# MingXiangL/SPE

Hardware: AMD Instinct MI355X
Metric: images/sec (whole node) at 3x800x1333 bs=2/GPU (higher is better)
Workload: dtype bf16/fp16 operands, fp32 accumulate; 1 GPU; TSCAM_cait_S24 (C=384, depth 24, 8 heads) + 0-layer encoder + 6-layer conditional-DETR decoder x2 stages, 100 queries, COCO heads (91), 2x3x800x1333 per GPU (N=4150 tokens), fwd + SetCriterion + SetCriterionRefine + bwd + grad all-reduce + clip + AdamW; global_batch=2, parallelism=dp1

## Files before the change

include/spe_hip.h:

```cpp
#ifndef SPE_HIP_H
#define SPE_HIP_H
#include <stddef.h>
#include <stdint.h>

#ifdef __cplusplus
extern "C" {
#endif

typedef struct ihipStream_t* spe_stream_t;

int spe_abi_version(void);

int spe_set_reduce_workspace(void* ws, size_t bytes, spe_stream_t stream);
int spe_reduce_defer_ranges(const void* const* ptrs, const size_t* bytes, int n);
int spe_reduce_defer_arena(void* arena, size_t bytes);
int spe_reduce_flush(spe_stream_t stream);
int spe_reduce_pending(void);

int spe_gemm_f32(const float* A, const float* B, float* C, const float* bias, float* C2,
                 int M, int N, int K, long lda, long ldb, long ldc, int transA, int transB,
                 int batch0, int batch1, long sA0, long sA1, long sB0, long sB1, long sC0, long sC1,
                 float alpha, int act, int splitk, int precision, spe_stream_t stream);

int spe_gemm_ex(const void* A, int a_bf16, const float* B, float* C, const float* bias, float* C2,
// ... 28 lines not shown
                               float* const* db, int R, int nblk, int N, int K, spe_stream_t stream);
int spe_gemm_bf16tn(const void* A16, const void* B16, float* C, int M, int N, int R, long lda, long ldb, long ldc,
                    float alpha, int splitk, spe_stream_t stream);
int spe_gemm_bf16tn_plan(int M, int N, int R, long lda, long ldb, int splitk, int* v);
int spe_gemm_bf16nt_ex(const void* A16, const void* B16, const void* A16lo, const void* B16lo, float* C, const float* bias,
                       float* C2, void* out16, void* out16lo, long ld16, void* out16T, long ld16t, float* colsum, const float* aux,
                       const float* res, const float* rgamma, int M, int N, int K, long lda, long ldb, long ldc, float alpha, int act,
                       int half_flags, spe_stream_t stream);
int spe_gemm_bf16nt_exd(const void* A16, const void* B16, const void* A16lo, const void* B16lo, float* C, const float* bias,
                        float* C2, void* out16, void* out16lo, long ld16, void* out16T, long ld16t, float* colsum, const float* aux,
                        const float* res, const float* rgamma, int M, int N, int K, long lda, long ldb, long ldc, float alpha, int act,
                        int half_flags, float p_drop, uint64_t seed, uint64_t offset, const float* sample_scale, long rows_per_sample,
                        spe_stream_t stream);
int spe_gemm_bf16nt_plan(int M, int N, int K, int split, int ex, int f16_operands, int f16_second, int splitk, int has_out16t,
                         long ld16t, int* plan);
int spe_cvt_bf16(const float* x, long ldx, int R, int C, void* out, void* out_lo, long ldo, void* outT, long ldt, float* colsum,
                 const float* aux, int act, spe_stream_t stream);
int spe_cvt_bf16_h(const float* x, long ldx, int R, int C, void* out, void* out_h, long ldo, void* outT, long ldt, spe_stream_t stream);
int spe_cvt_bf16_multi(const void* jobs_dev, int njobs, int total_tiles, spe_stream_t stream);

int spe_softmax_fwd(const float* S, const unsigned char* mask, float* P, float* Pd, int B, int H, int Nq,
                    int Nk, long ld, float p_drop, uint64_t seed, uint64_t offset, spe_stream_t stream);
int spe_softmax_bwd(const float* dPd, const float* P, float* dS, int B, int H, int Nq, int Nk, long ld,
                    float p_drop, uint64_t seed, uint64_t offset, spe_stream_t stream);

int spe_talking_softmax_fwd(const float* S, const float* Wl, const float* bl, const float* Ww, const float* bw,
                            float* P, float* Pd, int B, int H, int Nq, int Nk, long ld, float p_drop,
                            uint64_t seed, uint64_t offset, spe_stream_t stream);
int spe_talking_softmax_bwd(const float* dPd, const float* P, const float* S, const float* Wl, const float* Ww,
                            float* dS, float* ws, int nblocks, int B, int H, int Nq, int Nk, long ld,
// ... 158 lines not shown
```

spe_amd/csrc/gemm_bf16.hip:

```cpp
#include <cstdlib>
#include "common.h"
#include "gemm16_epilogue.h"
#include "det_reduce.h"
#include "gemm_nt_select.h"
#include "gemm_tiles.h"

template <int R>
__device__ __forceinline__ void g16_load(const unsigned short* __restrict__ base, long ld, int row0, int nrows, int k0, int K,
                                         u32x4g_t (&v)[R / 32]) {
    const int t = threadIdx.x;
    const int k = k0 + (t & 7) * 8;
    const bool kv = k < K;
    const int kc = kv ? k : 0;
#pragma unroll
    for (int i = 0; i < R / 32; ++i) {
        const int r = min(row0 + (t >> 3) + 32 * i, nrows - 1);
        const u32x4g_t q = *reinterpret_cast<const u32x4g_t*>(base + (long)r * ld + kc);
        v[i] = kv ? q : (u32x4g_t){0u, 0u, 0u, 0u};
    }
}
template <int R>
__device__ __forceinline__ void g16_stage(unsigned short* lds, const u32x4g_t (&v)[R / 32]) {
    const int t = threadIdx.x;
#pragma unroll
// ... 233 lines not shown
    p.out16 = nullptr; p.out16T = nullptr; p.colsum = nullptr; p.aux = nullptr; p.ld16 = 0; p.ld16t = 0; p.res = nullptr; p.rgamma = nullptr;
    p.drop_p = 0.f; p.drop_seed = p.drop_off = 0; p.sscale = nullptr; p.rps = 1;
    const int ktiles = (K + GB_BK - 1) / GB_BK;
    if (p.h16 && (splitk != 1 || C2 || (ldc & 3))) return -2;
    if ((p.h16 & 1) && A16lo) return -2;
    if (splitk < 0) {
        splitk = -splitk; p.slab = (long)M * ldc;
        if (splitk > ktiles) return -5;
    } else if (splitk > 1) return -2;
    if (splitk < 1) splitk = 1;
    p.kt_per_split = (ktiles + splitk - 1) / splitk;
    p.splitk = splitk;
    if (splitk > 1 && (act != 0 || C2 != nullptr || bias != nullptr)) return -3;
    if (p.Alo && splitk != 1) return -3;
    return nt_gemm_launch(p, false, stream);
}

static int gemm_bf16nt_ex_impl(const void* A16, const void* B16, const void* A16lo, const void* B16lo, float* C, const float* bias,
                               float* C2, void* out16, void* out16lo, long ld16, void* out16T, long ld16t, float* colsum,
                               const float* aux, const float* res, const float* rgamma,
                               int M, int N, int K, long lda, long ldb, long ldc, float alpha, int act, int half_flags,
                               float p_drop, uint64_t seed, uint64_t offset, const float* sample_scale, long rows_per_sample, hipStream_t stream);
extern "C" int spe_gemm_bf16nt_ex(const void* A16, const void* B16, const void* A16lo, const void* B16lo, float* C, const float* bias,
                                  float* C2, void* out16, void* out16lo, long ld16, void* out16T, long ld16t, float* colsum,
                                  const float* aux, const float* res, const float* rgamma,
                                  int M, int N, int K, long lda, long ldb, long ldc, float alpha, int act, int half_flags, hipStream_t stream) {
    return gemm_bf16nt_ex_impl(A16, B16, A16lo, B16lo, C, bias, C2, out16, out16lo, ld16, out16T, ld16t, colsum, aux, res, rgamma, M, N, K, lda, ldb,
                               ldc, alpha, act, half_flags, 0.f, 0, 0, nullptr, 1, stream);
}
extern "C" int spe_gemm_bf16nt_exd(const void* A16, const void* B16, const void* A16lo, const void* B16lo, float* C, const float* bias,
// ... 194 lines not shown
```

spe_amd/csrc/gemm_nt2.hip:

```cpp
#include <cstdlib>
#include "common.h"
#include "gemm16_epilogue.h"
#include "gemm_nt_select.h"
#include "gemm_tiles.h"

template <int CPR>
__device__ __forceinline__ int nt2_swz(int r) {
    if constexpr (CPR == 8) return r & 7;
    else return (0x78 >> (2 * ((r >> 2) & 3))) & 3;
}

template <int BM, int BN, int BK, int NST, bool SPLIT, bool EX, bool F16>
__global__ __launch_bounds__(256, 2) void gemm_nt2_kernel(Gemm16Args p) {
    extern __shared__ __attribute__((aligned(16))) unsigned short smem16[];
    constexpr int NFM = BM / 32, NFN = BN / 32, WM = BM / 2, WN = BN / 2;
    constexpr int CPR = BK / 8;
    constexpr int RPP = 64 / CPR;
    constexpr int PA = BM / RPP, PB = BN / RPP;
    constexpr int NP = (PA + PB) * (SPLIT ? 2 : 1), PW = NP / 4;
    constexpr int STE = NP * 512;
    static_assert(NP % 4 == 0 && BM % 32 == 0 && BN % 32 == 0 && (BK == 32 || BK == 64) && NST >= 2, "tile geometry");

    const int tiles_m = (p.M + BM - 1) / BM, tiles_n = (p.N + BN - 1) / BN;
    int tm, tn;
    if (!tile_decode(p.xcd_bind, tiles_m, tiles_n, tm, tn)) return;
    const int m0 = tm * BM, n0 = tn * BN;
    if (p.stagger > 0 && (blockIdx.x >> 8) == 1) {
        for (int i = 0; i < p.stagger; ++i) __builtin_amdgcn_s_sleep(127);
// ... 82 lines not shown
                        typedef _Float16 nt2_h8_t __attribute__((ext_vector_type(8)));
                        acc[i][j] = __builtin_amdgcn_mfma_f32_16x16x32_f16(__builtin_bit_cast(nt2_h8_t, b[j]), __builtin_bit_cast(nt2_h8_t, a[i]), acc[i][j], 0, 0, 0);
                    } else acc[i][j] = __builtin_amdgcn_mfma_f32_16x16x32_bf16(b[j], a[i], acc[i][j], 0, 0, 0);
                }
        }
    }
    asm volatile("s_waitcnt vmcnt(0)" ::: "memory");
    __syncthreads();
#if defined(SPE_ABLATE) && defined(SPE_ABL_NOSTORE)
#pragma unroll
    for (int i = 0; i < NFM; ++i)
#pragma unroll
        for (int j = 0; j < NFN; ++j) asm volatile("" :: "v"(acc[i][j]));
    return;
#endif
    if constexpr (EX) gemm16_epilogue_ex<BM, BN, SPLIT || F16, false>(p, acc, smem16, m0, n0);
    else if (F16 && (p.h16 & 2) && (p.N & 7) == 0 && (p.ldc & 7) == 0) gemm16_epilogue_h16<BM, BN>(p, acc, smem16, m0, n0);
    else gemm16_epilogue_plain<BM, BN>(p, acc, p.C, m0, n0);
}

template <int BM, int BN, int BK, int NST, bool SPLIT, bool EX, bool F16>
int launch_nt2(const Gemm16Args& p, hipStream_t stream) {
    constexpr int ring = NST * ((BM + BN) / (64 / (BK / 8))) * (SPLIT ? 2 : 1) * 1024;
    constexpr int epi = EX ? BM * (BN + 8) * 2 * ((SPLIT || F16) ? 2 : 1) : 0;
    constexpr int smem = ring > epi ? ring : epi;
    static bool attr_set = false;
    if (!attr_set) {
        hipError_t e = hipFuncSetAttribute(reinterpret_cast<const void*>(&gemm_nt2_kernel<BM, BN, BK, NST, SPLIT, EX, F16>),
                                           hipFuncAttributeMaxDynamicSharedMemorySize, smem);
        if (e != hipSuccess) return (int)e;
        attr_set = true;
// ... 2 lines not shown
    const TileOrder order = tile_order(p.M, p.N, tiles_m, tiles_n);
    Gemm16Args q = p;
    q.xcd_bind = order.xcd_bind;
    q.stagger = 0;
    const DetDeferSeg sg[1] = {{q.colsum, q.N}};
    float* region = (EX && q.colsum) ? det_defer_try(tiles_n, tiles_m, BN, 1, sg, stream) : nullptr;
    if (region) q.ws.defer = region;
    hipLaunchKernelGGL((gemm_nt2_kernel<BM, BN, BK, NST, SPLIT, EX, F16>), dim3(order.grid), dim3(256), smem, stream, q);
    if (region) det_defer_commit(region, tiles_n, tiles_m, BN, 1, sg, 1);
    SPE_CHECK_LAUNCH();
    return 0;
}
#define NT2_INSTANTIATE(BM, BN, BK, NST, SPLIT, EX, F16) template int launch_nt2<BM, BN, BK, NST, SPLIT, EX, F16>(const Gemm16Args&, hipStream_t);
NT2_INSTANCES(NT2_INSTANTIATE)
#undef NT2_INSTANTIATE
```

spe_amd/csrc/gemm_nt_select.h:

```cpp
#pragma once

enum NtFamily { NT_FAMILY_NT2 = 0, NT_FAMILY_BF16NT = 1 };

struct NtProblem {
    int M, N, K;
    bool split;
    bool ex;
    bool f16;
    bool f16_second;
    int splitk;
    bool out16t;
    long ld16t;
};

struct NtPlan {
    int err;
    int family;
    int BM, BN, BK;
    int NST;
    int NTS;
    bool SPLIT, EX, F16;
};

constexpr int NT2_MIN_ROWS = 2048;
// ... 58 lines not shown
}

#define NT2_INSTANCES(X)                                                                                                      \
    X(128, 128, 64, 2, false, true, true)   X(128, 64, 64, 2, false, true, true)                                              \
    X(160, 128, 64, 2, false, false, true)  X(128, 128, 64, 2, false, false, true)                                            \
    X(160, 128, 32, 2, true, false, false)  X(160, 128, 64, 2, false, false, false)                                           \
    X(64, 64, 64, 2, false, false, false)   X(64, 64, 64, 2, false, true, false)                                              \
    X(128, 64, 32, 2, true, false, false)   X(128, 64, 32, 2, true, true, false)                                              \
    X(128, 128, 32, 2, true, false, false)  X(128, 128, 32, 2, true, true, false)                                             \
    X(128, 128, 64, 2, false, false, false) X(128, 128, 64, 2, false, true, false)
#define BF16NT_INSTANCES(X)                                                                                                   \
    X(128, 128, false, 0, false) X(128, 128, true, 0, false) X(128, 64, false, 0, false) X(128, 64, true, 0, false)           \
    X(64, 64, false, 0, false)   X(64, 64, true, 0, false)   X(64, 64, false, 0, true)   X(64, 64, true, 0, true)             \
    X(64, 64, false, 6, false)   X(64, 64, false, 7, false)

constexpr int nt_key(int family, int BM, int BN, int BK, int NST, int NTS, bool SPLIT, bool EX, bool F16) {
    return (((((((family * 256 + BM) * 256 + BN) * 2 + (BK == 64)) * 4 + NST) * 8 + NTS) * 2 + SPLIT) * 2 + EX) * 2 + F16;
}
inline int nt_key(const NtPlan& s) { return nt_key(s.family, s.BM, s.BN, s.BK, s.NST, s.NTS, s.SPLIT, s.EX, s.F16); }
```

spe_amd/kernels.py:

```python
import ctypes
import os

import torch

from . import lib

_PRECISION = 2
import functools as _functools
import threading as _threading

_TLS = _threading.local()


def _in_bwd():
    return getattr(_TLS, "in_bwd", False)


def backward_scope(fn):
    @_functools.wraps(fn)
    def wrapped(ctx, *grads):
        prev, _TLS.in_bwd = _in_bwd(), True
        if _DEFER_FLATS is not None and not _FLUSH_QUEUED[0]:
            _FLUSH_QUEUED[0] = True
            try:
# ... 497 lines not shown

def linear_res_fwd(x2, W, b, res, gamma, save=True, src=None, drop=None, sscale=None, rps=1):
    R, K = x2.shape
    N = W.shape[0]
    dev = x2.device
    sp = split_fwd()
    x16, x16lo = act16(x2, src, want_lo=sp)
    out = torch.empty((R, N), device=dev, dtype=torch.float32)
    y = torch.empty((R, N), device=dev, dtype=torch.float16 if MLP_PRE_F16 else torch.float32) if save else None
    Wt = weight16(W, lo=sp)
    gemm16_ex(x16, Wt[0], R, N, K, K, K, bias=b, C=out, C2=y, res=res, rgamma=gamma, Alo=x16lo, Blo=Wt[2] if sp else None,
              drop=drop, sscale=sscale, rps=rps)
    return out, (x16, y)


def linear_res_bwd(dout2, saved, W, gamma, need_dx=True, grad_bufs=(None, None, None), drop=None, sscale=None, rps=1, pre=None):
    x16, y = saved
    R, N = dout2.shape
    K = W.shape[1]
    gW, gb, gg = grad_bufs
    if pre is not None:
        dy16, db, dg = pre
    else:
        dy16, _, db, dg = layerscale_residual_bwd16(dout2, y, gamma, ((R + 63) // 64) * 64, db_out=gb, dg_out=gg, want_rowmajor=True, want_T=False,
                                                    drop=drop, sscale=sscale, rps=rps)
    dW = _dw16_tn(dy16, x16, N, K, R, gW)
    dx = None
    if need_dx:
        dx = torch.empty((R, K), device=dout2.device, dtype=torch.float32)
        gemm16(dy16, weight16(W)[1], dx, R, K, N, N, N, K)
    return dx, dW, db, dg


MLP_PRE_F16 = False


MLP_F16 = True


def gemm16_plan(M, N, K, split=False, ex=False, op_f16=False, lo_f16=False, splitk=1, out16T=False, ld16t=0):
    v = (ctypes.c_int * 9)()
    rc = lib.load().spe_gemm_bf16nt_plan(M, N, K, int(split), int(ex), int(op_f16), int(lo_f16), int(splitk), int(out16T), int(ld16t), v)
    if rc != 0:
        return None
# ... 517 lines not shown
            shape = (B, H, nt, (dh + 31) // 32, 64, 8)
        else:
            shape = (B, H, nt, (dh + 15) // 16, 64, 4)
        outs.append(torch.empty(shape, device=x4.device, dtype=torch.float16 if kind >= F16 else torch.bfloat16))
    xs = (ctypes.c_void_p * n)(*[j[0].data_ptr() for j in jobs])
    strides = (ctypes.c_long * (3 * n))(*[s for j in jobs for s in (j[0].stride(0), j[0].stride(1), j[0].stride(2))])
    scales = (ctypes.c_float * n)(*[float(j[1]) for j in jobs])
    kinds = (ctypes.c_int * n)(*[{32: 0, 16: 1, 322: 2}[j[2] % F16] + (16 if j[2] >= F16 else 0) for j in jobs])
    optr = (ctypes.c_void_p * n)(*[o.data_ptr() for o in outs])
    Ns = (ctypes.c_int * n)(*[j[0].shape[1] for j in jobs])
    dhs = (ctypes.c_int * n)(*[j[0].shape[3] for j in jobs])
    _call("spe_attn_pack_multi", n, xs, strides, scales, kinds, optr, Ns, dhs, B, H, _st())
    return outs


def mha_plan(B, H, Lq, Lk):
    nch = ctypes.c_int(0)
    lib.call("spe_mha_plan", B, H, Lq, Lk, ctypes.byref(nch))
    return nch.value


def mha_fwd(Qf, Kf, V16, mask_u8, B, H, Lq, Lk, dk, dv, nch, p_drop, seed, offset):
    dev = Qf.device
    ntq, ntk, dvt = (Lq + 15) // 16, (Lk + 15) // 16, (dv + 15) // 16
    items = B * H * ntq * nch
    opart = torch.empty((items, dvt, 64, 4), device=dev, dtype=torch.float32)
    ml = torch.empty((items, 16, 2), device=dev, dtype=torch.float32)
    O = torch.empty((B, Lq, H * dv), device=dev, dtype=torch.float32)
    lse = torch.empty((B, H, Lq), device=dev, dtype=torch.float32)
    keep = torch.empty((B * H * ntq * ntk * 4,), device=dev, dtype=torch.int64) if p_drop > 0 else None
# ... 473 lines not shown
```

spe_amd/models/cait.py:

```python
from functools import partial

import torch
import torch.nn as nn
import torch.nn.functional as F

from .. import kernels as K
from .. import ops
from .layers import Dropout, LayerNorm, Linear, trunc_normal_

_REGISTRY = {}


def register_model(fn):
    _REGISTRY[fn.__name__] = fn
    return fn


def create_model(name, pretrained=False, **kwargs):
    if name not in _REGISTRY:
        raise RuntimeError(f"Unknown backbone {name!r}; available: {sorted(_REGISTRY)}")
    kwargs = {k: v for k, v in kwargs.items() if v is not None}
    return _REGISTRY[name](pretrained=pretrained, **kwargs)


# ... 62 lines not shown
        self.attn = Attention_block(dim, num_heads=num_heads, qkv_bias=qkv_bias, qk_scale=qk_scale,
                                    attn_drop=attn_drop, proj_drop=drop)
        self.drop_path = float(drop_path)
        self.norm2 = norm_layer(dim)
        self.mlp = Mlp_block(in_features=dim, hidden_features=int(dim * mlp_ratio), drop=drop)
        self.gamma_1 = nn.Parameter(init_values * torch.ones(dim))
        self.gamma_2 = nn.Parameter(init_values * torch.ones(dim))

    def forward(self, x, single_out=False, acc=None):
        B = x.shape[0]
        skip = isinstance(self.norm1, LayerNorm) and isinstance(self.norm2, LayerNorm)
        ss1 = ops.drop_path_scale(B, self.drop_path, self.training, x.device)
        y, xs = self.norm1.skip(x) if skip else (self.norm1(x), x)
        if isinstance(self.attn, Attention_talking_head):
            x = ops.linear_residual(self.attn.context(y, acc), self.attn.proj.weight, self.attn.proj.bias, xs, self.gamma_1, ss1,
                                    self.attn.proj_drop.p if self.training else 0.0, single=skip)
        else:
            assert acc is None, "the attention-map accumulator needs Attention_talking_head"
            x = ops.layerscale_residual(xs, self.attn(y), self.gamma_1, ss1)
        ss = ops.drop_path_scale(B, self.drop_path, self.training, x.device)
        mlp16 = isinstance(self.mlp, Mlp) and x.is_cuda and K.mlp_f16_ok(x.numel() // x.shape[-1], x.shape[-1], self.mlp.fc1.weight.shape[0],
                                                                        self.mlp.fc2.weight.shape[0])
        y, xs = self.norm2.skip(x, mlp16) if skip else (self.norm2(x), x)
        if isinstance(self.mlp, Mlp):
            return ops.mlp_gelu_residual(y, self.mlp.fc1.weight, self.mlp.fc1.bias, self.mlp.fc2.weight,
                                         self.mlp.fc2.bias, xs, self.gamma_2, ss, self.mlp.drop.p if self.training else 0.0, single=single_out)
        return ops.layerscale_residual(xs, self.mlp(y), self.gamma_2, ss)


def _skip_norms(blk):
    return isinstance(blk, LayerScale_Block) and isinstance(blk.norm1, LayerNorm) and isinstance(blk.norm2, LayerNorm)
# ... 365 lines not shown
```

spe_amd/ops.py:

```python
import os

import torch
from torch.autograd import Function

from . import kernels as K

ACT_NONE, ACT_RELU, ACT_GELU = 0, 1, 2


class _Linear(Function):

    @staticmethod
    @K.forward_scope
    def forward(ctx, x, W, b, act):
        shp = x.shape
        x2 = x.reshape(-1, shp[-1])
        if not x2.is_contiguous():
            x2 = x2.contiguous()
        Wc = W if W.is_contiguous() else W.contiguous()
        y, pre, xsave = K.linear_fwd(x2, Wc, b, act, want_pre=(act == ACT_GELU), save_for_dw=ctx.needs_input_grad[1], src=x)
        aux = pre if act == ACT_GELU else (y if act == ACT_RELU else None)
        ctx.act = act
        ctx.has_bias = b is not None
        ctx.params = (W, b)
# ... 407 lines not shown
    def forward(ctx, qkv, Wl, bl, Ww, bw, H, scale, p_drop, acc=None):
        train = any(ctx.needs_input_grad)
        O, saved = _TalkingHeadsAttentionFused._fwd(ctx, qkv, Wl, bl, Ww, bw, H, scale, p_drop, train, acc)
        if train:
            ctx.save_for_backward(*saved)
        return O

    @staticmethod
    def _fwd(ctx, qkv, Wl, bl, Ww, bw, H, scale, p_drop, train, acc=None):
        B, N, C3 = qkv.shape
        C = C3 // 3
        dh = C // H
        qkv = qkv.contiguous()
        v5 = qkv.view(B, N, 3, H, dh)
        q, k, v = v5[:, :, 0], v5[:, :, 1], v5[:, :, 2]
        nt = (N + 15) // 16
        jobs = [(q, scale * K.LOG2E, 32 + K.F16), (k, 1.0, 32 + K.F16), (v, 1.0, 16 + K.F16)]
        if train:
            jobs += [(v, 1.0, 32), (k, 1.0, 16), (q, 1.0, 16)]
        packed = K.attn_pack_multi(jobs)
        Qf, Kf, V16 = packed[:3]
        Wl, bl, Ww, bw = Wl.contiguous(), bl.contiguous(), Ww.contiguous(), bw.contiguous()
        seed, off = K.next_rng() if p_drop > 0 else (0, 0)
        _, _, c0 = K.talking_row_constants(Qf, Kf, Wl, bl, B, H, N, dh)
        want16 = K.produces16(B * N, C)
        if acc is not None:
            K.attn_pmean(Qf, Kf, Wl, c0, acc[0], acc[1], B, H, N, dh)
        O, O16, O16lo, bits = K.talking_flash_fwd(Qf, Kf, V16, Wl, Ww, bw, c0, B, H, N, dh, p_drop, seed, off, want16, K.split_fwd(),
                                                  want_bits=True)
        if O16 is not None:
            K.attach16(O, O16, O16lo)
        ctx.meta = (B, N, C, H, dh, nt, scale, p_drop)
        ctx.wparams = (Wl, bl, Ww, bw)
        ctx.has_bits = train and bits is not None
        saved = (packed[3], packed[4], packed[5], Qf, Kf, c0, Wl, Ww, bw) + ((bits,) if ctx.has_bits else ()) if train else ()
        return O, saved

    @staticmethod
    @K.backward_scope
    def backward(ctx, dO):
        return (*_TalkingHeadsAttentionFused._bwd(ctx, ctx.saved_tensors, dO, False), None, None, None, None)

    @staticmethod
    def _bwd(ctx, saved, dO, out16):
        Vf, K16, Q16, Qf, Kf, c0, Wl, Ww, bw = saved[:9]
        kbits = saved[9] if ctx.has_bits else None
        B, N, C, H, dh, nt, scale, p_drop = ctx.meta
        dO = dO.contiguous()
        dqkv = torch.empty((B, N, 3 * C), device=dO.device, dtype=torch.bfloat16 if out16 else torch.float32)
        d5 = dqkv.view(B, N, 3, H, dh)
        dq, dk, dv = d5[:, :, 0], d5[:, :, 1], d5[:, :, 2]
        f32 = (lambda t: None) if out16 else (lambda t: t)
        b16 = (lambda t: t) if out16 else (lambda t: None)
        dO4 = dO.view(B, N, H, dh)
        dOf, dO16 = K.attn_pack_multi([(dO4, 1.0, 32), (dO4, 1.0, 16)])
        dS = K.score_blocks(B, H, N, dO.device)
        Drows, ws_w = K.talking_bwdk_pass1(Qf, dOf, dO16, Kf, Vf, Wl, Ww, bw, c0, kbits, f32(dv), b16(dv), B, H, N, dh, p_drop)
        K.talking_bwdq_pass2(Qf, dOf, Kf, Vf, K16, Wl, Ww, c0, Drows, ws_w, dS, f32(dq), b16(dq), scale, kbits, B, H, N, dh, p_drop)
        dWl, dbl, dWw, dbw = K.talking_wgrad_reduce(ws_w, H, ctx.wparams)
        K.attn_contract(dS, Q16, f32(dk), True, alpha=scale, out16=b16(dk))
        return dqkv, dWl, dbl, dWw, dbw


class _QkvTalkingAttention(Function):

    @staticmethod
    @K.forward_scope
    def forward(ctx, x, Wq, bq, Wl, bl, Ww, bw, H, scale, p_drop, acc=None):
        shp = x.shape
        x2 = x.reshape(-1, shp[-1])
        if not x2.is_contiguous():
            x2 = x2.contiguous()
        y, _, xsave = K.linear_fwd(x2, Wq, bq, 0, want_pre=False, save_for_dw=True, src=x)
        O, saved = _TalkingHeadsAttentionFused._fwd(ctx, y.view(*shp[:-1], Wq.shape[0]), Wl, bl, Ww, bw, H, scale, p_drop, True, acc)
        ctx.qparams = (Wq, bq)
        ctx.save_for_backward(xsave, *saved)
        return O

    @staticmethod
    @K.backward_scope
    def backward(ctx, dO):
        xsave, *saved = ctx.saved_tensors
        Wq, bq = ctx.qparams
        d16, dWl, dbl, dWw, dbw = _TalkingHeadsAttentionFused._bwd(ctx, saved, dO, True)
        N3, Kd = Wq.shape
        R = d16.numel() // N3
        d16 = d16.view(R, N3)
        dev = d16.device
        gb = K.grad_buffer(bq)
        db = gb.view(-1) if gb is not None else torch.empty((N3,), device=dev, dtype=torch.float32)
        K.colsum_bf16_blocks(d16, N3, [db])
        dW = K._dw16_tn(d16, xsave, N3, Kd, R, K.grad_buffer(Wq)) if ctx.needs_input_grad[1] else None
        dx = None
        if ctx.needs_input_grad[0]:
            dx = torch.empty((R, Kd), device=dev, dtype=torch.float32)
            K.gemm16(d16, K.weight16(Wq)[1], dx, R, Kd, N3, N3, N3, Kd)
            dx = dx.view(*dO.shape[:-1], Kd)
        return dx, dW, db.view_as(bq), dWl, dbl, dWw, dbw, None, None, None, None


def qkv_talking_attention_ok(x, Wq, bq, num_heads):
    C = x.shape[-1]
    R = x.numel() // C
    return (x.is_cuda and bq is not None and Wq.is_contiguous() and torch.is_grad_enabled()
            and (x.requires_grad or Wq.requires_grad) and Wq.requires_grad and bq.requires_grad
            and K.get_precision() != "bf16x3" and K._lin16_ok(R, Wq.shape[0], C) and not K._lin_small_ok(R, Wq.shape[0], C)
            and K.fused_supported(num_heads, C // num_heads))


def qkv_talking_attention(x, Wq, bq, Wl, bl, Ww, bw, num_heads, scale, p_drop=0.0, acc=None):
    return _QkvTalkingAttention.apply(x, Wq, bq, Wl, bl, Ww, bw, num_heads, scale, p_drop, acc)


class _MlpGelu(Function):

# ... 15 lines not shown
    @K.backward_scope
    def backward(ctx, dy):
        x16, pre, h16, W1, W2 = ctx.saved_tensors
        dy2 = dy.reshape(-1, W2.shape[0])
        if not dy2.is_contiguous():
            dy2 = dy2.contiguous()
        bufs = tuple(K.grad_buffer(p) for p in ctx.params)
        dx, dW1, db1, dW2, db2 = K.mlp_gelu_bwd(dy2, (x16, pre, h16), W1, W2, ctx.needs_input_grad[0], bufs)
        return (dx.view(*dy.shape[:-1], W1.shape[1]) if dx is not None else None), dW1, db1, dW2, db2


class _LinearRes(Function):

    @staticmethod
    @K.forward_scope
    def forward(ctx, x, W, b, xres, gamma, sscale=None, p_drop=0.0, single=False):
        shp = x.shape
        x2 = x.reshape(-1, shp[-1])
        if not x2.is_contiguous():
            x2 = x2.contiguous()
        r2 = xres.reshape(-1, xres.shape[-1])
        if not r2.is_contiguous():
            r2 = r2.contiguous()
        train = any(ctx.needs_input_grad)
        ctx.drop = (float(p_drop), *K.next_rng()) if p_drop > 0 else None
        ctx.ls_single = bool(single and train and p_drop <= 0 and sscale is None and not K.MLP_PRE_F16 and W.requires_grad
                             and b.requires_grad and gamma.requires_grad)
        ctx.ls_done = None
        ctx.rps = r2.shape[0] // xres.shape[0]
        out, saved = K.linear_res_fwd(x2, W, b, r2, gamma, save=train, src=x, drop=ctx.drop, sscale=sscale, rps=ctx.rps)
        ctx.params = (W, b, gamma)
        ctx.has_ss = sscale is not None
        if train:
            ctx.save_for_backward(*saved, W, gamma, *((sscale,) if sscale is not None else ()))
        return out.view(xres.shape)

    @staticmethod
    @K.backward_scope
    def backward(ctx, dout):
        x16, y, W, gamma = ctx.saved_tensors[:4]
        ss = ctx.saved_tensors[4] if ctx.has_ss else None
        d2 = dout.reshape(-1, W.shape[0])
        if not d2.is_contiguous():
            d2 = d2.contiguous()
        pre = _ls_taken(ctx, dout if dout.is_contiguous() else d2)
        bufs = tuple(K.grad_buffer(p) for p in ctx.params)
        dx, dW, db, dg = K.linear_res_bwd(d2, (x16, y), W, gamma, ctx.needs_input_grad[0], bufs, drop=ctx.drop, sscale=ss, rps=ctx.rps, pre=pre)
        return (dx.view(*dout.shape[:-1], W.shape[1]) if dx is not None else None), dW, db, dout, dg.view_as(gamma), None, None, None

def _ls_args(prod):
    sv = prod.saved_tensors
    if prod._forward_cls is _LinearRes:
        return sv[1], sv[3], prod.params[1], prod.params[2]
    return sv[3], sv[6], prod.params[3], prod.params[4]


def _ls_taken(ctx, d2):
    done = getattr(ctx, "ls_done", None)
    if done is None:
        return None
    ctx.ls_done = None
    pre, ptr, ver = done
    if d2.data_ptr() != ptr or d2._version != ver:
        raise RuntimeError("spe_amd.ops: a node was marked single=True but its output had more than one consumer (the LayerNorm backward already "
                           "accumulated its bias / LayerScale gradients from a partial gradient)")
    return pre


FUSE_DROP = True


def linear_residual(x, W, b, xres, gamma, sample_scale=None, p_drop=0.0, single=False):
    R = x.numel() // x.shape[-1]
    N, Kd = W.shape
    if ((FUSE_DROP or (sample_scale is None and p_drop <= 0)) and b is not None and W.is_contiguous()
            and gamma.is_contiguous() and N % 4 == 0 and N <= 1024 and K._lin16_ok(R, N, Kd)
            and (sample_scale is None or (sample_scale.is_contiguous() and R % xres.shape[0] == 0))):
        return _LinearRes.apply(x, W, b, xres, gamma, sample_scale, p_drop, single)
    return layerscale_residual(xres, dropout(linear(x, W, b), p_drop, p_drop > 0), gamma, sample_scale)


class _MlpGeluRes(Function):

    @staticmethod
    @K.forward_scope
    def forward(ctx, x, W1, b1, W2, b2, xres, gamma, sscale=None, p_drop=0.0, single=False):
        shp = x.shape
        x2 = x.reshape(-1, shp[-1])
        if not x2.is_contiguous():
            x2 = x2.contiguous()
        r2 = xres.reshape(-1, xres.shape[-1])
        if not r2.is_contiguous():
            r2 = r2.contiguous()
# ... 466 lines not shown
```

Before: 41.67 images/sec.

## Emit attention fragment records directly from QKV and proj-backward GEMM epilogues

Adds a record-writing epilogue to the nt2 bf16 GEMM kernel so it scatters outputs straight into the packed per-head fragment layouts the fused talking-heads attention consumes. The forward QKV projection now writes Q/K/V records directly instead of materialising qkv and then running a separate pack pass. In backward, the proj layer's dx GEMM writes the dO records for the attention backward, so the dO pack pass and the dense dx write are skipped. This relies on a single-consumer assumption, guarded by a pointer/version check, and only a fixed set of tile configurations is supported.

```diff
diff --git a/include/spe_hip.h b/include/spe_hip.h
--- a/include/spe_hip.h
+++ b/include/spe_hip.h
@@ -66,6 +66,9 @@
                         spe_stream_t stream);
 int spe_gemm_bf16nt_plan(int M, int N, int K, int split, int ex, int f16_operands, int f16_second, int splitk, int has_out16t,
                          long ld16t, int* plan);
+int spe_gemm_bf16nt_rec(const void* A16, const void* B16, const void* A16lo, const void* B16lo, const float* bias, int M, int N, int K,
+                        long lda, long ldb, float alpha, int B_img, int N_tok, int H, int dh, int nout, void* const* outs,
+                        const int* thirds, const int* kinds, const float* scales, spe_stream_t stream);
 int spe_cvt_bf16(const float* x, long ldx, int R, int C, void* out, void* out_lo, long ldo, void* outT, long ldt, float* colsum,
                  const float* aux, int act, spe_stream_t stream);
 int spe_cvt_bf16_h(const float* x, long ldx, int R, int C, void* out, void* out_h, long ldo, void* outT, long ldt, spe_stream_t stream);
diff --git a/spe_amd/csrc/gemm_bf16.hip b/spe_amd/csrc/gemm_bf16.hip
--- a/spe_amd/csrc/gemm_bf16.hip
+++ b/spe_amd/csrc/gemm_bf16.hip
@@ -1,6 +1,7 @@
 #include <cstdlib>
 #include "common.h"
 #include "gemm16_epilogue.h"
+#include "gemm_rec_epilogue.h"
 #include "det_reduce.h"
 #include "gemm_nt_select.h"
 #include "gemm_tiles.h"
@@ -271,6 +272,49 @@
     if (splitk > 1 && (act != 0 || C2 != nullptr || bias != nullptr)) return -3;
     if (p.Alo && splitk != 1) return -3;
     return nt_gemm_launch(p, false, stream);
+}
+
+template <int BM, int BN, int BK, int NST, bool SPLIT>
+int launch_nt2_rec(const Gemm16Args& p, const RecArgs& ra, hipStream_t stream);
+
+extern "C" int spe_gemm_bf16nt_rec(const void* A16, const void* B16, const void* A16lo, const void* B16lo, const float* bias, int M, int N, int K,
+                                   long lda, long ldb, float alpha, int B_img, int N_tok, int H, int dh, int nout, void* const* outs,
+                                   const int* thirds, const int* kinds, const float* scales, hipStream_t stream) {
+    if (M <= 0 || N <= 0 || K <= 0 || B_img <= 0 || N_tok <= 0 || H <= 0 || dh <= 0 || nout <= 0 || nout > REC_MAXOUT) return -2;
+    auto al16 = [](const void* q) { return (reinterpret_cast<uintptr_t>(q) & 15) == 0; };
+    if (!al16(A16) || !al16(B16) || !al16(A16lo) || !al16(B16lo) || (lda & 7) || (ldb & 7) || (K & 7)) return -2;
+    if ((A16lo != nullptr) != (B16lo != nullptr)) return -2;
+    const long C = (long)H * dh;
+    if ((dh & 15) || (long)B_img * N_tok != M || N % C != 0 || N / C > 3) return -2;
+    RecArgs ra;
+    ra.N_tok = N_tok; ra.H = H; ra.dh = dh;
+    for (int t = 0; t < 3; ++t) ra.t[t] = RecThird{nullptr, nullptr, 0.f, 0.f, 0, 0};
+    for (int i = 0; i < nout; ++i) {
+        if (!outs[i] || (reinterpret_cast<uintptr_t>(outs[i]) & 7) || thirds[i] < 0 || thirds[i] >= N / C || (kinds[i] & ~17)) return -2;
+        RecThird& rt = ra.t[thirds[i]];
+        if (kinds[i] & 1) {
+            if (rt.o16) return -2;
+            rt.o16 = outs[i]; rt.s16 = scales[i]; rt.h16 = (kinds[i] >> 4) & 1;
+        } else {
+            if (rt.o32) return -2;
+            rt.o32 = outs[i]; rt.s32 = scales[i]; rt.h32 = (kinds[i] >> 4) & 1;
+        }
+    }
+    Gemm16Args p;
+    p.A = reinterpret_cast<const unsigned short*>(A16); p.B = reinterpret_cast<const unsigned short*>(B16);
+    p.Alo = reinterpret_cast<const unsigned short*>(A16lo); p.Blo = reinterpret_cast<const unsigned short*>(B16lo); p.out16lo = nullptr;
+    p.C = nullptr; p.C2 = nullptr; p.bias = bias; p.M = M; p.N = N; p.K = K; p.lda = lda; p.ldb = ldb; p.ldc = N;
+    p.h16 = 0; p.alpha = alpha; p.act = 0; p.slab = 0; p.splitk = 1; p.kt_per_split = (K + GB_BK - 1) / GB_BK;
+    p.ws = DetWs{nullptr, nullptr, 0, 0}; p.half_flags = 0;
+    p.out16 = nullptr; p.out16T = nullptr; p.colsum = nullptr; p.aux = nullptr; p.ld16 = 0; p.ld16t = 0; p.res = nullptr; p.rgamma = nullptr;
+    p.drop_p = 0.f; p.drop_seed = p.drop_off = 0; p.sscale = nullptr; p.rps = 1;
+    const NtPlan s = nt_gemm_select(nt_problem(p, false));
+    if (s.err || s.family != NT_FAMILY_NT2 || s.EX || s.F16) return -2;
+#define NT2_REC_CASE(bm, bn, bk, nst, split) \
+    if (s.BM == bm && s.BN == bn && s.BK == bk && s.NST == nst && s.SPLIT == split) return launch_nt2_rec<bm, bn, bk, nst, split>(p, ra, stream);
+    NT2_REC_INSTANCES(NT2_REC_CASE)
+#undef NT2_REC_CASE
+    return -2;
 }
 
 static int gemm_bf16nt_ex_impl(const void* A16, const void* B16, const void* A16lo, const void* B16lo, float* C, const float* bias,
diff --git a/spe_amd/csrc/gemm_nt2.hip b/spe_amd/csrc/gemm_nt2.hip
--- a/spe_amd/csrc/gemm_nt2.hip
+++ b/spe_amd/csrc/gemm_nt2.hip
@@ -1,6 +1,7 @@
 #include <cstdlib>
 #include "common.h"
 #include "gemm16_epilogue.h"
+#include "gemm_rec_epilogue.h"
 #include "gemm_nt_select.h"
 #include "gemm_tiles.h"
 
@@ -10,8 +11,9 @@
     else return (0x78 >> (2 * ((r >> 2) & 3))) & 3;
 }
 
-template <int BM, int BN, int BK, int NST, bool SPLIT, bool EX, bool F16>
-__global__ __launch_bounds__(256, 2) void gemm_nt2_kernel(Gemm16Args p) {
+template <int BM, int BN, int BK, int NST, bool SPLIT, bool EX, bool F16, class... REC>
+__global__ __launch_bounds__(256, 2) void gemm_nt2_kernel(Gemm16Args p, REC... ra) {
+    static_assert(sizeof...(REC) == 0 || (sizeof...(REC) == 1 && !EX && !F16), "at most one RecArgs, on the plain bf16 product");
     extern __shared__ __attribute__((aligned(16))) unsigned short smem16[];
     constexpr int NFM = BM / 32, NFN = BN / 32, WM = BM / 2, WN = BN / 2;
     constexpr int CPR = BK / 8;
@@ -124,7 +126,8 @@
         for (int j = 0; j < NFN; ++j) asm volatile("" :: "v"(acc[i][j]));
     return;
 #endif
-    if constexpr (EX) gemm16_epilogue_ex<BM, BN, SPLIT || F16, false>(p, acc, smem16, m0, n0);
+    if constexpr (sizeof...(REC) > 0) gemm16_epilogue_rec<BM, BN>(p, ra..., acc, smem16, m0, n0);
+    else if constexpr (EX) gemm16_epilogue_ex<BM, BN, SPLIT || F16, false>(p, acc, smem16, m0, n0);
     else if (F16 && (p.h16 & 2) && (p.N & 7) == 0 && (p.ldc & 7) == 0) gemm16_epilogue_h16<BM, BN>(p, acc, smem16, m0, n0);
     else gemm16_epilogue_plain<BM, BN>(p, acc, p.C, m0, n0);
 }
@@ -157,3 +160,27 @@
 #define NT2_INSTANTIATE(BM, BN, BK, NST, SPLIT, EX, F16) template int launch_nt2<BM, BN, BK, NST, SPLIT, EX, F16>(const Gemm16Args&, hipStream_t);
 NT2_INSTANCES(NT2_INSTANTIATE)
 #undef NT2_INSTANTIATE
+
+template <int BM, int BN, int BK, int NST, bool SPLIT>
+int launch_nt2_rec(const Gemm16Args& p, const RecArgs& ra, hipStream_t stream) {
+    constexpr int ring = NST * ((BM + BN) / (64 / (BK / 8))) * (SPLIT ? 2 : 1) * 1024;
+    static_assert(BM * (BN + 8) * 2 <= ring, "the staged 16-bit tile of the record epilogue lives in the operand ring");
+    static bool attr_set = false;
+    if (!attr_set) {
+        hipError_t e = hipFuncSetAttribute(reinterpret_cast<const void*>(&gemm_nt2_kernel<BM, BN, BK, NST, SPLIT, false, false, RecArgs>),
+                                           hipFuncAttributeMaxDynamicSharedMemorySize, ring);
+        if (e != hipSuccess) return (int)e;
+        attr_set = true;
+    }
+    const int tiles_m = (p.M + BM - 1) / BM, tiles_n = (p.N + BN - 1) / BN;
+    const TileOrder order = tile_order(p.M, p.N, tiles_m, tiles_n);
+    Gemm16Args q = p;
+    q.xcd_bind = order.xcd_bind;
+    q.stagger = 0;
+    hipLaunchKernelGGL((gemm_nt2_kernel<BM, BN, BK, NST, SPLIT, false, false, RecArgs>), dim3(order.grid), dim3(256), ring, stream, q, ra);
+    SPE_CHECK_LAUNCH();
+    return 0;
+}
+#define NT2_REC_INSTANTIATE(BM, BN, BK, NST, SPLIT) template int launch_nt2_rec<BM, BN, BK, NST, SPLIT>(const Gemm16Args&, const RecArgs&, hipStream_t);
+NT2_REC_INSTANCES(NT2_REC_INSTANTIATE)
+#undef NT2_REC_INSTANTIATE
diff --git a/spe_amd/csrc/gemm_nt_select.h b/spe_amd/csrc/gemm_nt_select.h
--- a/spe_amd/csrc/gemm_nt_select.h
+++ b/spe_amd/csrc/gemm_nt_select.h
@@ -96,6 +96,10 @@
     X(64, 64, false, 0, false)   X(64, 64, true, 0, false)   X(64, 64, false, 0, true)   X(64, 64, true, 0, true)             \
     X(64, 64, false, 6, false)   X(64, 64, false, 7, false)
 
+#define NT2_REC_INSTANCES(X)                                                                                                  \
+    X(160, 128, 32, 2, true)  X(160, 128, 64, 2, false)  X(128, 128, 32, 2, true)  X(128, 128, 64, 2, false)                  \
+    X(128, 64, 32, 2, true)   X(64, 64, 64, 2, false)
+
 constexpr int nt_key(int family, int BM, int BN, int BK, int NST, int NTS, bool SPLIT, bool EX, bool F16) {
     return (((((((family * 256 + BM) * 256 + BN) * 2 + (BK == 64)) * 4 + NST) * 8 + NTS) * 2 + SPLIT) * 2 + EX) * 2 + F16;
 }
diff --git a/spe_amd/csrc/gemm_rec_epilogue.h b/spe_amd/csrc/gemm_rec_epilogue.h
--- /dev/null
+++ b/spe_amd/csrc/gemm_rec_epilogue.h
@@ -0,0 +1,104 @@
+#pragma once
+#include "attn_pack.h"
+#include "gemm16_epilogue.h"
+
+#define REC_MAXOUT 6
+struct RecThird {
+    void* o32; void* o16;
+    float s32, s16;
+    int h32, h16;
+};
+struct RecArgs { RecThird t[3]; int N_tok, H, dh; };
+
+template <int BM, int BN>
+__device__ __forceinline__ void gemm16_epilogue_rec(const Gemm16Args& p, const RecArgs& ra, f32x4_t (&acc)[BM / 32][BN / 32], unsigned short* smem16,
+                                                    const int m0, const int n0) {
+    constexpr int NFM = BM / 32, NFN = BN / 32, WM = BM / 2, WN = BN / 2, LR = BN + 8;
+    const int lane = threadIdx.x & 63, w = __builtin_amdgcn_readfirstlane(threadIdx.x >> 6);
+    const int wm = w >> 1, wn = w & 1;
+    const int fr = lane & 15, fc = lane >> 4;
+    const int Nt = ra.N_tok, H = ra.H, dh = ra.dh, C = H * dh, nt = (Nt + 15) >> 4;
+    const FragGeom fg = frag_geom(dh);
+    const int full = fg.full;
+    const long rec8 = fg.rec8;
+    long rrec[NFM]; int rr[NFM]; bool rowv[NFM], lastr[NFM];
+#pragma unroll
+    for (int i = 0; i < NFM; ++i) {
+        const int m = m0 + wm * WM + i * 16 + fr, mc = min(m, p.M - 1);
+        const int b = mc / Nt, r = mc - b * Nt;
+        rowv[i] = m < p.M; rr[i] = r & 15; rrec[i] = ((long)b * H * nt + (r >> 4)) * rec8; lastr[i] = rowv[i] && r == Nt - 1;
+    }
+#pragma unroll
+    for (int j = 0; j < NFN; ++j) {
+        const int nf = n0 + wn * WN + j * 16;
+        if (nf >= p.N) continue;
+        const int third = nf / C, cf = nf - third * C, h = cf / dh, d = cf - h * dh + fc * 4, nl = wn * WN + j * 16 + fc * 4, n = n0 + nl;
+        const RecThird rt = ra.t[third];
+        float bv[4] = {0.f, 0.f, 0.f, 0.f};
+        if (p.bias) {
+#pragma unroll
+            for (int r = 0; r < 4; ++r) bv[r] = p.bias[n + r];
+        }
+        const long hrec = (long)h * nt * rec8;
+        const bool instep = d < 32 * full;
+        const int u32 = instep ? (d >> 5) * 128 + 32 * ((d & 31) >> 3) + ((d & 7) >> 2) : full * 128 + 16 * ((d - 32 * full) >> 2);
+        const int mul = instep ? 2 : 1;
+#pragma unroll
+        for (int i = 0; i < NFM; ++i) {
+            float v[4];
+#pragma unroll
+            for (int r = 0; r < 4; ++r) v[r] = acc[i][j][r] * p.alpha;
+#pragma unroll
+            for (int r = 0; r < 4; ++r) v[r] += bv[r];
+            if (!rowv[i]) continue;
+            if (rt.o32) {
+                uint2* dst = reinterpret_cast<uint2*>(rt.o32) + rrec[i] + hrec + u32;
+                dst[mul * rr[i]] = spe_cvt4_16(v[0] * rt.s32, v[1] * rt.s32, v[2] * rt.s32, v[3] * rt.s32, rt.h32);
+                if (lastr[i])
+                    for (int e = rr[i] + 1; e < 16; ++e) dst[mul * e] = make_uint2(0u, 0u);
+            }
+            if (rt.o16)
+                *reinterpret_cast<uint2*>(smem16 + (wm * WM + i * 16 + fr) * LR + nl) =
+                    spe_cvt4_16(v[0] * rt.s16, v[1] * rt.s16, v[2] * rt.s16, v[3] * rt.s16, rt.h16);
+        }
+    }
+    if (!ra.t[0].o16 && !ra.t[1].o16 && !ra.t[2].o16) return;
+    asm volatile("s_waitcnt lgkmcnt(0)" ::: "memory");
+    __builtin_amdgcn_s_barrier();
+    asm volatile("" ::: "memory");
+    const int mend = min(m0 + BM, p.M);
+    const int c16 = lane & 15, qs = lane >> 4;
+    for (int cg = w; cg < BN / 16; cg += 4) {
+        const int nf = n0 + cg * 16;
+        if (nf >= p.N) break;
+        const int third = nf / C, cf = nf - third * C, h = cf / dh, d = cf - h * dh + c16, nl = cg * 16 + c16;
+        unsigned short* out = reinterpret_cast<unsigned short*>(ra.t[third].o16);
+        if (!out) continue;
+        for (int b = m0 / Nt; b <= (mend - 1) / Nt; ++b) {
+            const int base = b * Nt;
+            const int lo = max(m0, base) - base, hi = min(mend, base + Nt) - base;
+            const bool owns_last = hi == Nt;
+            const int qend = owns_last ? 4 * nt : (hi + 3) >> 2;
+            unsigned short* orec = out + ((((long)b * H + h) * nt) * rec8 + (d >> 4) * 64 + (d & 15)) * 4;
+            for (int q = ((lo >> 2) & ~3) + qs; q < qend; q += 4) {
+                if (4 * q + 3 < lo) continue;
+                unsigned short e[4]; bool mine[4];
+#pragma unroll
+                for (int k = 0; k < 4; ++k) {
+                    const int r = 4 * q + k;
+                    const bool data = r >= lo && r < hi;
+                    mine[k] = data || (owns_last && r >= Nt);
+                    const unsigned short s = smem16[min(max(base + r - m0, 0), BM - 1) * LR + nl];
+                    e[k] = data ? s : (unsigned short)0;
+                }
+                unsigned short* dst = orec + ((q >> 2) * rec8 + 16 * (q & 3)) * 4;
+                if (mine[0] && mine[1] && mine[2] && mine[3])
+                    *reinterpret_cast<uint2*>(dst) = make_uint2((unsigned)e[0] | ((unsigned)e[1] << 16), (unsigned)e[2] | ((unsigned)e[3] << 16));
+                else {
+#pragma unroll
+                    for (int k = 0; k < 4; ++k) if (mine[k]) dst[k] = e[k];
+                }
+            }
+        }
+    }
+}
diff --git a/spe_amd/kernels.py b/spe_amd/kernels.py
--- a/spe_amd/kernels.py
+++ b/spe_amd/kernels.py
@@ -535,7 +535,7 @@
     return out, (x16, y)
 
 
-def linear_res_bwd(dout2, saved, W, gamma, need_dx=True, grad_bufs=(None, None, None), drop=None, sscale=None, rps=1, pre=None):
+def linear_res_bwd(dout2, saved, W, gamma, need_dx=True, grad_bufs=(None, None, None), drop=None, sscale=None, rps=1, pre=None, rec=None):
     x16, y = saved
     R, N = dout2.shape
     K = W.shape[1]
@@ -549,6 +549,10 @@
     dx = None
     if need_dx:
         dx = torch.empty((R, K), device=dout2.device, dtype=torch.float32)
+        if rec is not None:
+            B_img, N_tok, H, dh = rec
+            recs = gemm16_records(dy16, weight16(W)[1], R, K, N, N, N, B_img, N_tok, H, dh, [(0, 1.0, 32), (0, 1.0, 16)])
+            return dx, dW, db, dg, recs
         gemm16(dy16, weight16(W)[1], dx, R, K, N, N, N, K)
     return dx, dW, db, dg
 
@@ -1096,6 +1100,49 @@
     return outs
 
 
+QKV_RECORDS = True
+_REC_TILES = {(160, 128, 32, True), (160, 128, 64, False), (128, 128, 32, True), (128, 128, 64, False), (128, 64, 32, True), (64, 64, 64, False)}
+
+
+@_functools.lru_cache(maxsize=None)
+def _rec_tile_ok(M, N, Kd, split):
+    p = gemm16_plan(M, N, Kd, split=split)
+    return p is not None and p["family"] == "nt2" and (p["BM"], p["BN"], p["BK"], p["SPLIT"]) in _REC_TILES
+
+
+def gemm_records_ok(R, N, Kd, H, dh, split):
+    return (QKV_RECORDS and R >= 2048 and Kd % 64 == 0 and dh % 16 == 0 and N % (H * dh) == 0 and N // (H * dh) <= 3 and fused_supported(H, dh)
+            and _rec_tile_ok(R, N, Kd, bool(split)))
+
+
+def gemm16_records(A16, B16, M, N, Kd, lda, ldb, B_img, N_tok, H, dh, jobs, bias=None, Alo=None, Blo=None, alpha=1.0):
+    n = len(jobs)
+    nt = (N_tok + 15) // 16
+    outs = []
+    for _, _, kind in jobs:
+        shape = (B_img, H, nt, frag_record_elems(dh)) if kind % F16 == 32 else (B_img, H, nt, (dh + 15) // 16, 64, 4)
+        outs.append(torch.empty(shape, device=A16.device, dtype=torch.float16 if kind >= F16 else torch.bfloat16))
+    optr = (ctypes.c_void_p * n)(*[o.data_ptr() for o in outs])
+    thirds = (ctypes.c_int * n)(*[int(j[0]) for j in jobs])
+    kinds = (ctypes.c_int * n)(*[{32: 0, 16: 1}[j[2] % F16] + (16 if j[2] >= F16 else 0) for j in jobs])
+    scales = (ctypes.c_float * n)(*[float(j[1]) for j in jobs])
+    _call("spe_gemm_bf16nt_rec", _p(A16), _p(B16), _p(Alo), _p(Blo), _p(bias), M, N, Kd, lda, ldb, float(alpha), B_img, N_tok, H, dh, n, optr,
+          thirds, kinds, scales, _st())
+    return outs
+
+
+def qkv_records_fwd(x2, W, b, B_img, N_tok, H, dh, scale, train, src=None):
+    R, Kd = x2.shape
+    N = W.shape[0]
+    sp = split_fwd()
+    x16, x16lo = act16(x2, src, want_lo=sp)
+    Wt = weight16(W, lo=sp)
+    jobs = [(0, scale * LOG2E, 32 + F16), (1, 1.0, 32 + F16), (2, 1.0, 16 + F16)]
+    if train:
+        jobs += [(2, 1.0, 32), (1, 1.0, 16), (0, 1.0, 16)]
+    return gemm16_records(x16, Wt[0], R, N, Kd, Kd, Kd, B_img, N_tok, H, dh, jobs, bias=b, Alo=x16lo, Blo=Wt[2] if sp else None), x16
+
+
 def mha_plan(B, H, Lq, Lk):
     nch = ctypes.c_int(0)
     lib.call("spe_mha_plan", B, H, Lq, Lk, ctypes.byref(nch))
diff --git a/spe_amd/models/cait.py b/spe_amd/models/cait.py
--- a/spe_amd/models/cait.py
+++ b/spe_amd/models/cait.py
@@ -100,7 +100,7 @@
         y, xs = self.norm1.skip(x) if skip else (self.norm1(x), x)
         if isinstance(self.attn, Attention_talking_head):
             x = ops.linear_residual(self.attn.context(y, acc), self.attn.proj.weight, self.attn.proj.bias, xs, self.gamma_1, ss1,
-                                    self.attn.proj_drop.p if self.training else 0.0, single=skip)
+                                    self.attn.proj_drop.p if self.training else 0.0, single=skip, x_single=True)
         else:
             assert acc is None, "the attention-map accumulator needs Attention_talking_head"
             x = ops.layerscale_residual(xs, self.attn(y), self.gamma_1, ss1)
diff --git a/spe_amd/ops.py b/spe_amd/ops.py
--- a/spe_amd/ops.py
+++ b/spe_amd/ops.py
@@ -445,11 +445,16 @@
         qkv = qkv.contiguous()
         v5 = qkv.view(B, N, 3, H, dh)
         q, k, v = v5[:, :, 0], v5[:, :, 1], v5[:, :, 2]
-        nt = (N + 15) // 16
         jobs = [(q, scale * K.LOG2E, 32 + K.F16), (k, 1.0, 32 + K.F16), (v, 1.0, 16 + K.F16)]
         if train:
             jobs += [(v, 1.0, 32), (k, 1.0, 16), (q, 1.0, 16)]
-        packed = K.attn_pack_multi(jobs)
+        return _TalkingHeadsAttentionFused._fwd_records(ctx, K.attn_pack_multi(jobs), (B, N, C), Wl, bl, Ww, bw, H, scale, p_drop, train, acc)
+
+    @staticmethod
+    def _fwd_records(ctx, packed, shape, Wl, bl, Ww, bw, H, scale, p_drop, train, acc=None):
+        B, N, C = shape
+        dh = C // H
+        nt = (N + 15) // 16
         Qf, Kf, V16 = packed[:3]
         Wl, bl, Ww, bw = Wl.contiguous(), bl.contiguous(), Ww.contiguous(), bw.contiguous()
         seed, off = K.next_rng() if p_drop > 0 else (0, 0)
@@ -473,18 +478,20 @@
         return (*_TalkingHeadsAttentionFused._bwd(ctx, ctx.saved_tensors, dO, False), None, None, None, None)
 
     @staticmethod
-    def _bwd(ctx, saved, dO, out16):
+    def _bwd(ctx, saved, dO, out16, dO_records=None):
         Vf, K16, Q16, Qf, Kf, c0, Wl, Ww, bw = saved[:9]
         kbits = saved[9] if ctx.has_bits else None
         B, N, C, H, dh, nt, scale, p_drop = ctx.meta
-        dO = dO.contiguous()
         dqkv = torch.empty((B, N, 3 * C), device=dO.device, dtype=torch.bfloat16 if out16 else torch.float32)
         d5 = dqkv.view(B, N, 3, H, dh)
         dq, dk, dv = d5[:, :, 0], d5[:, :, 1], d5[:, :, 2]
         f32 = (lambda t: None) if out16 else (lambda t: t)
         b16 = (lambda t: t) if out16 else (lambda t: None)
-        dO4 = dO.view(B, N, H, dh)
-        dOf, dO16 = K.attn_pack_multi([(dO4, 1.0, 32), (dO4, 1.0, 16)])
+        if dO_records is not None:
+            dOf, dO16 = dO_records
+        else:
+            dO4 = dO.contiguous().view(B, N, H, dh)
+            dOf, dO16 = K.attn_pack_multi([(dO4, 1.0, 32), (dO4, 1.0, 16)])
         dS = K.score_blocks(B, H, N, dO.device)
         Drows, ws_w = K.talking_bwdk_pass1(Qf, dOf, dO16, Kf, Vf, Wl, Ww, bw, c0, kbits, f32(dv), b16(dv), B, H, N, dh, p_drop)
         K.talking_bwdq_pass2(Qf, dOf, Kf, Vf, K16, Wl, Ww, c0, Drows, ws_w, dS, f32(dq), b16(dq), scale, kbits, B, H, N, dh, p_drop)
@@ -502,8 +509,14 @@
         x2 = x.reshape(-1, shp[-1])
         if not x2.is_contiguous():
             x2 = x2.contiguous()
-        y, _, xsave = K.linear_fwd(x2, Wq, bq, 0, want_pre=False, save_for_dw=True, src=x)
-        O, saved = _TalkingHeadsAttentionFused._fwd(ctx, y.view(*shp[:-1], Wq.shape[0]), Wl, bl, Ww, bw, H, scale, p_drop, True, acc)
+        C = Wq.shape[0] // 3
+        ctx.do_records = None
+        if x.dim() == 3 and K.gemm_records_ok(x2.shape[0], 3 * C, x2.shape[1], H, C // H, K.split_fwd()):
+            packed, xsave = K.qkv_records_fwd(x2, Wq, bq, shp[0], shp[1], H, C // H, scale, True, src=x)
+            O, saved = _TalkingHeadsAttentionFused._fwd_records(ctx, packed, (shp[0], shp[1], C), Wl, bl, Ww, bw, H, scale, p_drop, True, acc)
+        else:
+            y, _, xsave = K.linear_fwd(x2, Wq, bq, 0, want_pre=False, save_for_dw=True, src=x)
+            O, saved = _TalkingHeadsAttentionFused._fwd(ctx, y.view(*shp[:-1], Wq.shape[0]), Wl, bl, Ww, bw, H, scale, p_drop, True, acc)
         ctx.qparams = (Wq, bq)
         ctx.save_for_backward(xsave, *saved)
         return O
@@ -513,7 +526,7 @@
     def backward(ctx, dO):
         xsave, *saved = ctx.saved_tensors
         Wq, bq = ctx.qparams
-        d16, dWl, dbl, dWw, dbw = _TalkingHeadsAttentionFused._bwd(ctx, saved, dO, True)
+        d16, dWl, dbl, dWw, dbw = _TalkingHeadsAttentionFused._bwd(ctx, saved, dO, True, _do_records_taken(ctx, dO))
         N3, Kd = Wq.shape
         R = d16.numel() // N3
         d16 = d16.view(R, N3)
@@ -530,6 +543,18 @@
         return dx, dW, db.view_as(bq), dWl, dbl, dWw, dbw, None, None, None, None
 
 
+def _do_records_taken(ctx, dO):
+    done = getattr(ctx, "do_records", None)
+    if done is None:
+        return None
+    ctx.do_records = None
+    recs, ptr, ver = done
+    if dO.data_ptr() != ptr or dO._version != ver:
+        raise RuntimeError("spe_amd.ops: a node was marked x_single=True but the attention output it consumes had more than one consumer (its "
+                           "gradient was written as fragment records only: another consumer's gradient was added to unwritten memory)")
+    return recs
+
+
 def qkv_talking_attention_ok(x, Wq, bq, num_heads):
     C = x.shape[-1]
     R = x.numel() // C
@@ -575,7 +600,7 @@
 
     @staticmethod
     @K.forward_scope
-    def forward(ctx, x, W, b, xres, gamma, sscale=None, p_drop=0.0, single=False):
+    def forward(ctx, x, W, b, xres, gamma, sscale=None, p_drop=0.0, single=False, x_single=False):
         shp = x.shape
         x2 = x.reshape(-1, shp[-1])
         if not x2.is_contiguous():
@@ -584,6 +609,12 @@
         if not r2.is_contiguous():
             r2 = r2.contiguous()
         train = any(ctx.needs_input_grad)
+        prod = x.grad_fn if (x_single and K.QKV_RECORDS and x.requires_grad and x.dim() == 3) else None
+        ctx.attn = None
+        if prod is not None and getattr(prod, "_forward_cls", None) is _QkvTalkingAttention:
+            Ba, Na, Ca, Ha, dha = prod.meta[:5]
+            if (Ba, Na, Ca) == tuple(shp) and K.gemm_records_ok(x2.shape[0], Ca, W.shape[0], Ha, dha, False):
+                ctx.attn = prod
         ctx.drop = (float(p_drop), *K.next_rng()) if p_drop > 0 else None
         ctx.ls_single = bool(single and train and p_drop <= 0 and sscale is None and not K.MLP_PRE_F16 and W.requires_grad
                              and b.requires_grad and gamma.requires_grad)
@@ -606,8 +637,15 @@
             d2 = d2.contiguous()
         pre = _ls_taken(ctx, dout if dout.is_contiguous() else d2)
         bufs = tuple(K.grad_buffer(p) for p in ctx.params)
+        attn = ctx.attn if ctx.needs_input_grad[0] else None
+        if attn is not None:
+            dx, dW, db, dg, recs = K.linear_res_bwd(d2, (x16, y), W, gamma, True, bufs, drop=ctx.drop, sscale=ss, rps=ctx.rps, pre=pre,
+                                                    rec=(attn.meta[0], attn.meta[1], attn.meta[3], attn.meta[4]))
+            dxv = dx.view(*dout.shape[:-1], W.shape[1])
+            attn.do_records = (recs, dxv.data_ptr(), dxv._version)
+            return dxv, dW, db, dout, dg.view_as(gamma), None, None, None, None
         dx, dW, db, dg = K.linear_res_bwd(d2, (x16, y), W, gamma, ctx.needs_input_grad[0], bufs, drop=ctx.drop, sscale=ss, rps=ctx.rps, pre=pre)
-        return (dx.view(*dout.shape[:-1], W.shape[1]) if dx is not None else None), dW, db, dout, dg.view_as(gamma), None, None, None
+        return (dx.view(*dout.shape[:-1], W.shape[1]) if dx is not None else None), dW, db, dout, dg.view_as(gamma), None, None, None, None
 
 def _ls_args(prod):
     sv = prod.saved_tensors
@@ -631,13 +669,13 @@
 FUSE_DROP = True
 
 
-def linear_residual(x, W, b, xres, gamma, sample_scale=None, p_drop=0.0, single=False):
+def linear_residual(x, W, b, xres, gamma, sample_scale=None, p_drop=0.0, single=False, x_single=False):
     R = x.numel() // x.shape[-1]
     N, Kd = W.shape
     if ((FUSE_DROP or (sample_scale is None and p_drop <= 0)) and b is not None and W.is_contiguous()
             and gamma.is_contiguous() and N % 4 == 0 and N <= 1024 and K._lin16_ok(R, N, Kd)
             and (sample_scale is None or (sample_scale.is_contiguous() and R % xres.shape[0] == 0))):
-        return _LinearRes.apply(x, W, b, xres, gamma, sample_scale, p_drop, single)
+        return _LinearRes.apply(x, W, b, xres, gamma, sample_scale, p_drop, single, x_single)
     return layerscale_residual(xres, dropout(linear(x, W, b), p_drop, p_drop > 0), gamma, sample_scale)
 
 
```

New measurement: 43.03 images/sec (median of 3 runs). 1.03x the previous value.
